# Bernat-C/MRI-Diffusion-SuperResolution

Hardware: AMD Instinct MI355X
Metric: MRI slices/sec (50-step DDIM, 256^2, bs=32) (higher is better)
Workload: dtype bf16; 1 GPU; configs[1]: 256x256 1-ch synthetic MRI slices -> 4x32x32 latents, SD-1.5-size UNet (859.5M params, random init) + rank-4 LoRA, 50-step DDIM, bs=32 per GPU; ddim_steps=50, parallelism=slice-sharded x1 (no collective), lora=explicit adapters, down-projection + rank-r update inside the projection GEMMs, tile_table=profiles/r03_tune_cache.tsv, hipgraph=True

## Files before the change

mri-diffusion-superresolution_amd/csrc/common.h:

```cpp
#pragma once
#include <hip/hip_runtime.h>
#include <stdint.h>
#include <string>

#include "lora_hr.h"

namespace mrisr {

typedef __bf16 bf16;
typedef __attribute__((ext_vector_type(8))) __bf16 bf16x8;
typedef __attribute__((ext_vector_type(4))) __bf16 bf16x4;
typedef __attribute__((ext_vector_type(4))) float f32x4;
typedef __attribute__((ext_vector_type(16))) float f32x16;

enum DType : int { DT_F32 = 0, DT_BF16 = 1, DT_F16 = 2, DT_I64 = 3 };

template <typename T> struct TypeTag;
template <> struct TypeTag<float> { static constexpr int id = DT_F32; };
template <> struct TypeTag<bf16> { static constexpr int id = DT_BF16; };

__device__ __forceinline__ float to_f32(float x) { return x; }
__device__ __forceinline__ float to_f32(bf16 x) { return (float)x; }
template <typename T> __device__ __forceinline__ T from_f32(float x);
template <> __device__ __forceinline__ float from_f32<float>(float x) { return x; }
// ... 97 lines not shown
    const float* lora_z = nullptr;
    const float* lora_b = nullptr;
    int lora_r = 0, lora_zld = 0, lora_secN = 1;
    const void* lora_a = nullptr;
    int lora_R = 0;
    float* lora_zout = nullptr;
    const float* ln_gamma = nullptr;
    const float* ln_beta = nullptr;
    float ln_eps = 1e-5f;
    const void* w8 = nullptr;
    const float* w_scale = nullptr;
    const void* lora_a8 = nullptr;
    const float* lora_a_scale = nullptr;
    int no_rp = 0;
    int group_m = 1;
    int dbg = 0;
    unsigned long long* stamps = nullptr;
};

template <typename T> int launch_gemm(const GemmArgs& g, hipStream_t st);
template <typename T> int launch_splitk_reduce(const GemmArgs& g, hipStream_t st);
const void* zero_page();
int init_zero_page();
int gemm_prepare();
struct MlpArgs {
    const void* x = nullptr; int ldx = 0, M = 0;
    const float* ln_gamma = nullptr; const float* ln_beta = nullptr; float ln_eps = 1e-5f;
    const void* w1 = nullptr; const float* b1 = nullptr;
    const void* w2p = nullptr; const float* b2 = nullptr;
    const void* resid = nullptr; int ldr = 0;
// ... 280 lines not shown
```

mri-diffusion-superresolution_amd/csrc/gemm.hip:

```cpp
#include "common.h"
#include "gemm_head.h"
#include "prof.h"

#include <cstdio>
#include <cstdlib>
#include <cstring>
#include <map>
#include <mutex>
#include <unordered_map>

namespace mrisr {

static void* g_zero_page = nullptr;
static constexpr size_t kZeroPageBytes = 128 * 1024;
const void* zero_page() { return g_zero_page; }
int init_zero_page() {
    if (g_zero_page) return 0;
    MRISR_CHECK_HIP(hipMalloc(&g_zero_page, kZeroPageBytes));
    MRISR_CHECK_HIP(hipMemset(g_zero_page, 0, kZeroPageBytes));
    return 0;
}

typedef const __attribute__((address_space(1))) void* gptr_t;
typedef __attribute__((address_space(3))) void* lptr_t;
// ... 172 lines not shown
template <int NFR>
__device__ __forceinline__ void preload_cols(const GemmArgs& g, int nbase, f32x4 (&pb)[NFR]) {
    const bool fold = g.rowvec && g.rowvec_div >= g.M;
#pragma unroll
    for (int i = 0; i < NFR; ++i) pb[i] = f32x4{0.f, 0.f, 0.f, 0.f};
    if (g.bias) {
#pragma unroll
        for (int i = 0; i < NFR; ++i) pb[i] = *reinterpret_cast<const f32x4*>(g.bias + min(nbase + i * 16, g.N - 4));
    }
    if (fold) {
#pragma unroll
        for (int i = 0; i < NFR; ++i) pb[i] += *reinterpret_cast<const f32x4*>(g.rowvec + min(nbase + i * 16, g.N - 4));
    }
}

template <typename T> struct Frag;
template <> struct Frag<bf16> { typedef bf16x8 type; };
template <> struct Frag<float> { typedef f32x4 type; };

__device__ __forceinline__ void mma(f32x4& acc, const bf16x8& w, const bf16x8& a) {
    acc = __builtin_amdgcn_mfma_f32_16x16x32_bf16(w, a, acc, 0, 0, 0);
}
__device__ __forceinline__ void mma(f32x4& acc, const f32x4& w, const f32x4& a) {
#pragma unroll
    for (int j = 0; j < 4; ++j) acc = __builtin_amdgcn_mfma_f32_16x16x4f32(w[j], a[j], acc, 0, 0, 0);
}

__device__ __forceinline__ void lds_poison(char* smem_base, int nthreads) {
    const unsigned bytes = ((const __attribute__((address_space(4))) unsigned*)__builtin_amdgcn_dispatch_ptr())[7];
    for (unsigned o = threadIdx.x * 16u; o + 16u <= bytes; o += (unsigned)nthreads * 16u)
        *reinterpret_cast<uint4*>(smem_base + o) = make_uint4(~0u, ~0u, ~0u, ~0u);
    __syncthreads();
}
static int gemm_flags_now();

static constexpr int kStampHdr = 8, kStampWgs = 1024, kStampSlotWords = kStampHdr + 8 * kStampWgs, kStampSlots = 256;
__device__ __forceinline__ unsigned long long* gemm_stamp_slot(const GemmArgs& g, bool header) {
    if (!g.stamps) return nullptr;
    const unsigned wg = blockIdx.x + gridDim.x * (blockIdx.y + gridDim.y * blockIdx.z);
    if (header && wg == 0 && threadIdx.x == 0) {
        g.stamps[0] = (unsigned long long)g.M; g.stamps[1] = (unsigned long long)g.N; g.stamps[2] = (unsigned long long)g.K;
        g.stamps[3] = (unsigned long long)gridDim.x * gridDim.y * gridDim.z;
        g.stamps[4] = (g.resid ? 1u : 0u) | (g.lora_a ? 2u : 0u) | (g.conv ? 4u : 0u) | (g.cs0 ? 8u : 0u);
        g.stamps[5] = (unsigned long long)g.splitk; g.stamps[6] = (unsigned long long)(unsigned)g.dbg; g.stamps[7] = 1ull;
    }
    return wg < (unsigned)kStampWgs ? g.stamps + kStampHdr + (size_t)wg * 8 : nullptr;
}
__device__ __forceinline__ unsigned long long* gemm_stamp_word(const GemmArgs& g, int k, bool header = false) {
    unsigned long long* const slot = gemm_stamp_slot(g, header);
    return slot ? slot + k : nullptr;
}
static_assert(kStampSlotWords == kStampHdr + 8 * kStampWgs, "a slot: the header, then 8 words for each of the first kStampWgs workgroups");

template <typename T, int BM, int BN, int WGM, int WGN>
__global__ __launch_bounds__(256) void gemm_kernel(const GemmArgs g, const char* __restrict__ zero) {
    constexpr int EB = sizeof(T);
    constexpr int CH = 16 / EB;
    constexpr int BK = 8 * CH;
// ... 205 lines not shown
#pragma unroll
    for (int i = 0; i < NF; ++i)
#pragma unroll
        for (int j = 0; j < MF; ++j) {
            const int m = m0 + wm0 + j * 16 + fr;
            const int n = n0 + wn0 + i * 16 + fg * 4;
            if (m < g.M && n < g.N) {
                float v[4] = {acc[i][j][0], acc[i][j][1], acc[i][j][2], acc[i][j][3]};
                epilogue4<T>(g, z, m, n, v, nullptr, nullptr, nullptr, false, true, nullptr, 0, 0, 0, pb[i]);
            }
        }
}

template <int BM, int BN, int NT = 256>
__device__ __forceinline__ void copy_out_tile(const GemmArgs& g, const bf16* otile, int pitch, int m0, int n0, int z, bool add_resid,
                                              unsigned long long* stamp_resid = nullptr) {
    __syncthreads();
    constexpr int CPR = BN / 8;
    bf16* out = reinterpret_cast<bf16*>(g.out) + (size_t)z * g.o_bs;
    const bf16* res = add_resid ? reinterpret_cast<const bf16*>(g.resid) + (size_t)z * g.o_bs : nullptr;
    constexpr int TOTAL = BM * CPR, IT = (TOTAL + NT - 1) / NT, BATCH = IT < 5 ? IT : 5;
    for (int it0 = 0; it0 < IT; it0 += BATCH) {
        bf16x8 rv[BATCH];
#pragma unroll
        for (int u = 0; u < BATCH; ++u) {
            const int idx = (int)threadIdx.x + (it0 + u) * NT;
            const int row = idx / CPR, ch = idx - row * CPR;
            const int m = m0 + row, n = n0 + ch * 8;
            if (res && idx < TOTAL && m < g.M && n + 8 <= g.N) rv[u] = *reinterpret_cast<const bf16x8*>(res + (size_t)m * g.ldr + n);
        }
        if (stamp_resid && it0 == 0 && threadIdx.x == 0) {
            if (res) asm volatile("s_waitcnt vmcnt(0)" ::: "memory");
            *stamp_resid = __builtin_readcyclecounter();
        }
#pragma unroll
        for (int u = 0; u < BATCH; ++u) {
            const int idx = (int)threadIdx.x + (it0 + u) * NT;
            const int row = idx / CPR, ch = idx - row * CPR;
            const int m = m0 + row, n = n0 + ch * 8;
            if (idx >= TOTAL || m >= g.M || n >= g.N) continue;
            const bf16* src = otile + row * pitch + ch * 8;
            bf16* dst = out + (size_t)m * g.ldo + n;
            if (n + 8 <= g.N) {
                bf16x8 v = *reinterpret_cast<const bf16x8*>(src);
                if (res) {
#pragma unroll
                    for (int e = 0; e < 8; ++e) v[e] = (bf16)((float)v[e] + (float)rv[u][e]);
// ... 38 lines not shown
            const int b = m / g.ntok, tok = m - b * g.ntok;
            *reinterpret_cast<bf16x8*>(base + (((size_t)b * g.nheads + h) * g.dpad + dd) * g.npad + tok) =
                *reinterpret_cast<const bf16x8*>(otile + col * P + tc * 8);
        }
    }
}

typedef __attribute__((address_space(3))) void* lds_ptr_t;
__device__ __forceinline__ __amdgpu_buffer_rsrc_t make_rsrc(const void* p, unsigned bytes) {
    return __builtin_amdgcn_make_buffer_rsrc(const_cast<void*>(p), 0, bytes, 0x00020000);
}
__device__ __forceinline__ void bl16(__amdgpu_buffer_rsrc_t r, char* lds_wave_base, unsigned voff, unsigned soff) {
    __builtin_amdgcn_raw_ptr_buffer_load_lds(r, (lds_ptr_t)lds_wave_base, 16, voff, soff, 0, 0);
}
#define BL_OOB 0x80000000u


__device__ __forceinline__ void pretouch_weights(const __amdgpu_buffer_rsrc_t& rw, long long w_bytes, char* scratch, int wave, int lane, int cap) {
    const int n_wg = (int)(gridDim.x * gridDim.y);
    const int wg = (int)(blockIdx.x + blockIdx.y * gridDim.x);
    const long long pieces = (w_bytes + 1023) >> 10;
    const int per_wg = (int)((pieces + n_wg - 1) / n_wg);
    const int per_wave = min((per_wg + 3) >> 2, cap);
    const long long first = (long long)wg * per_wg + (long long)wave * per_wave;
    for (int i = 0; i < per_wave; ++i) {
        const long long pc = first + i;
        const unsigned off = pc < pieces ? (unsigned)(pc << 10) + (unsigned)lane * 16u : BL_OOB;
        bl16(rw, scratch + ((wave * 2 + (i & 1)) << 10), off, 0u);
    }
}
// ... 218 lines not shown
                for (int it = 0; it < A_IT; ++it) bl16(rs, sb + (it * 256 + wave * 64) * 16, avo[it], chb);
            } else if (!second) {
#pragma unroll
                for (int it = 0; it < A_IT; ++it) bl16(ra0, sb + (it * 256 + wave * 64) * 16, avo[it], chb);
            } else {
#pragma unroll
                for (int it = 0; it < A_IT; ++it) bl16(ra1, sb + (it * 256 + wave * 64) * 16, avo[it], chb);
            }
            cc += BK;
            if (cc >= Ct && !tail) { cc = 0; ++tap; }
        }
    };
    auto stage = [&](int kt, int buf) { stage_w(kt, buf); stage_a(kt, buf); };
    (void)acb;
    if (kt_beg < kt_end) stage_a(kt_beg, 0);
    stamp(1);

    f32x4 acc[NF][MF];
#pragma unroll
    for (int i = 0; i < NF; ++i)
#pragma unroll
        for (int j = 0; j < MF; ++j) acc[i][j] = f32x4{0.f, 0.f, 0.f, 0.f};

    const int wm0 = (wave / WGN) * WTM, wn0 = (wave % WGN) * WTN;
    const int fr = lane & 15, fg = lane >> 4;
    const bool zwave = LORA && (wave % WGN) == 0;
    const bool lora_mma = LORA && g.lora_r == 4 && g.alpha == 1.0f && !(g.dbg & 8);
    bf16x8 lbf[NF];
    if (LORA) {
#pragma unroll
// ... 31 lines not shown
#pragma unroll
                for (int j = 0; j < MF; ++j) acc[i][j] = __builtin_amdgcn_mfma_f32_16x16x32_bf16(wf[i], af[j], acc[i][j], 0, 0, 0);
            if (LORA && zwave) {
                const bf16x8 lf = *reinterpret_cast<const bf16x8*>(sw + (BN + fr) * 128 + phys);
#pragma unroll
                for (int j = 0; j < MF; ++j) zacc[j] = __builtin_amdgcn_mfma_f32_16x16x32_bf16(lf, af[j], zacc[j], 0, 0, 0);
            }
        }
    };

    if constexpr (NSTAGE == 2) {
        if (kt_beg < kt_end) {
            asm volatile("s_waitcnt vmcnt(0)" ::: "memory");
            __syncthreads();
            stamp(2);
            int cur = 0;
            const bool halves = (g.dbg & 16384) != 0;
            for (int kt = kt_beg; kt < kt_end; ++kt) {
                const bool more = kt + 1 < kt_end;
                if (more) { if (halves) stage_w(kt + 1, cur ^ 1); else stage(kt + 1, cur ^ 1); }
                compute(cur, [&]() {
                    if (halves) {
                        __builtin_amdgcn_sched_barrier(0);
                        if (more) stage_a(kt + 1, cur ^ 1);
                        __builtin_amdgcn_sched_barrier(0);
                    }
                });
                asm volatile("s_waitcnt vmcnt(0)" ::: "memory");
                __syncthreads();
                cur ^= 1;
// ... 64 lines not shown
                    store4<float>(part + (size_t)m * g.N + n, v);
                }
            }
        if constexpr (NF * MF > 20) return;
        else {
            if (!g.sk_counters) return;
            if (!splitk_last_arriver<NF, MF>(g, acc, (unsigned)(z * gridDim.x + blockIdx.x), g.partial + (size_t)z * g.splitk * (size_t)g.M * g.N,
                                             m0 + wm0, n0 + wn0, fr, fg, smem))
                return;
        }
    }
    constexpr bool kRing = NSTAGE > 2;
    f32x4 pb[kRing ? 1 : NF];
    float pbr[kRing ? NF : 1][4];
    if constexpr (kRing) preload_cols<NF>(g, n0 + wn0 + fg * 4, pbr);
    else preload_cols<NF>(g, n0 + wn0 + fg * 4, pb);
    auto cols = [&](int i, float (&o)[4]) {
#pragma unroll
        for (int r = 0; r < 4; ++r) {
            if constexpr (kRing) o[r] = pbr[i][r];
            else o[r] = pb[i][r];
        }
    };
    stamp(4, true);
    if (g.act == ACT_GEGLU) {
        if constexpr (NF % 2 == 0) {
#pragma unroll
            for (int i = 0; i < NF; i += 2)
#pragma unroll
                for (int j = 0; j < MF; ++j) {
                    const int m = m0 + wm0 + j * 16 + fr;
// ... 49 lines not shown
#pragma unroll
            for (int j = 0; j < MF; ++j) {
                const int m = m0 + wm0 + j * 16 + fr;
                const int n = n0 + wn0 + i * 16 + fg * 4;
                if (m < g.M && n < g.N) {
                    float v[4] = {acc[i][j][0], acc[i][j][1], acc[i][j][2], acc[i][j][3]};
                    float pbi[4];
                    cols(i, pbi);
                    epilogue4<T>(g, z, m, n, v, nullptr, LORA && !lora_mma ? zlds + (m - m0) * 16 : nullptr,
                                 staged || (hstaged && !htr) ? otile + (m - m0) * OPITCH + (n - n0) : nullptr, resid_later, true,
                                 hstaged && htr ? otile : nullptr, m - m0, n - n0, BM + 8, pbi);
                }
            }
    }
    stamp(5);
    if (staged) copy_out_tile<BM, BN>(g, otile, OPITCH, m0, n0, z, resid_later, NSTAGE == 2 ? gemm_stamp_word(g, 6) : nullptr);
    else if (hstaged) copy_out_heads<BM, BN>(g, otile, m0, n0, htr);
    stamp(7);
}

template <int BM, int BN, int WGM, int WGN>
__global__ __launch_bounds__(256, 2) void gemm_halo_kernel(const GemmHead hd, const GemmArgs g) {
    typedef bf16 T;
    constexpr int BK = 64;
    constexpr int W_IT = BN / 32;
    constexpr int WTM = BM / WGM, WTN = BN / WGN;
    constexpr int MF = WTM / 16, NF = WTN / 16;
    constexpr int WSTAGE = BN * 128;
    constexpr int PIT_MAX = (BM >= 256 ? 13 : (BM >= 128 ? 9 : 6));
    static_assert(WGM * WGN == 4, "4 waves");
    extern __shared__ __attribute__((aligned(16))) char smem[];
// ... 93 lines not shown
    }

    auto stage_patch = [&](int ch) {
        const int cc = ch * BK;
        const bool second = cc >= (int)h.c0;
        const unsigned chb = (unsigned)(second ? cc - (int)h.c0 : cc) * 2;
#pragma unroll
        for (int it = 0; it < PIT_MAX; ++it) {
            if (it < pit) {
                if (!second) bl16(ra0, patch + (it * 256 + wave * 64) * 16, pvo0[it], chb);
                else bl16(ra1, patch + (it * 256 + wave * 64) * 16, pvo1[it], chb);
            }
        }
    };
    if (ch_beg < ch_end) stage_patch(ch_beg);
    stamp(1);

    const bool has_tail = (h.flags & GH_TAIL) != 0;
    const long long a_rows = has_tail ? (long long)g.B * Hd * Wd : 0ll;
    const void* const s0p = has_tail ? g.s0 : nullptr;
    const void* const s1p = has_tail ? g.s1 : nullptr;
    const __amdgpu_buffer_rsrc_t rs0 = make_rsrc(s0p ? s0p : (const void*)a0p, s0p ? (unsigned)min(a_rows * g.lds0 * 2, 0x7FFFFFFFll) : 0u);
    const __amdgpu_buffer_rsrc_t rs1 = make_rsrc(s1p ? s1p : (const void*)a0p, s1p ? (unsigned)min(a_rows * g.lds1 * 2, 0x7FFFFFFFll) : 0u);
    unsigned spix[PIT_MAX];
    auto sc_setup = [&]() {
#pragma unroll
        for (int it = 0; it < PIT_MAX; ++it) {
            int t = it * 256 + tid;
            asm volatile("" : "+v"(t));
            const int pp = t >> 3;
// ... 68 lines not shown
                for (int t = tid; t < npix * 8; t += 256) {
                    bf16x8 v = *reinterpret_cast<bf16x8*>(patch + t * 16);
#pragma unroll
                    for (int e = 0; e < 8; ++e) {
                        const float f = (float)v[e] * 1.0009765625f + 0.03125f;
                        v[e] = (bf16)(f / (1.0f + __expf(-f)));
                    }
                    *reinterpret_cast<bf16x8*>(patch + t * 16) = v;
                }
                __syncthreads();
            }
            for (int tap = 0; tap < 9; ++tap) {
                if (tap + 1 < 9) stage_w(ch, tap + 1, cur ^ 1);
                else if (ch + 1 < ch_end) stage_w(ch + 1, 0, cur ^ 1);
                else if (sc_beg < sc_end) stage_w_sc(sc_beg, cur ^ 1);
                compute(cur, tap);
                asm volatile("s_waitcnt vmcnt(0)" ::: "memory");
                __syncthreads();
                cur ^= 1;
            }
        }
        if (sc_beg < sc_end) sc_setup();
        for (int sc = sc_beg; sc < sc_end; ++sc) {
            stage_patch_sc(sc);
            asm volatile("s_waitcnt vmcnt(0)" ::: "memory");
            __syncthreads();
            if (sc + 1 < sc_end) stage_w_sc(sc + 1, cur ^ 1);
            compute(cur, 4);
            asm volatile("s_waitcnt vmcnt(0)" ::: "memory");
            __syncthreads();
// ... 14 lines not shown
                    float v[4] = {acc[i][j][0], acc[i][j][1], acc[i][j][2], acc[i][j][3]};
                    store4<float>(part + (size_t)m * g.N + n, v);
                }
            }
        if constexpr (NF * MF > 20) return;
        else {
            if (!g.sk_counters) return;
            if (!splitk_last_arriver<NF, MF>(g, acc, blockIdx.x, g.partial, m0 + wm0, n0 + wn0, fr, fg, smem)) return;
        }
    }
    constexpr int OPITCH = BN + 8;
    T* otile = reinterpret_cast<T*>(smem);
    const bool staged = g.out_mode == OUT_ROWS && (g.ldo & 7) == 0 && (size_t)BM * OPITCH * 2 <= (size_t)pit * 4096 + 2 * WSTAGE && g.stage_out > 1;
    const bool resid_later = staged && g.resid != nullptr && (g.ldr & 7) == 0 && g.stage_out < 3;
    f32x4 pb[NF];
    preload_cols<NF>(g, n0 + wn0 + fg * 4, pb);
    stamp(4, true);
    const bool plain_epi = !(g.dbg & 64) && staged && g.act == ACT_NONE && !g.lora_z && (!g.resid || resid_later);
    if (plain_epi) {
        const float alpha = g.alpha;
        const bool rows_rv = g.rowvec && g.rowvec_div < g.M;
#pragma unroll
        for (int i = 0; i < NF; ++i)
#pragma unroll
            for (int j = 0; j < MF; ++j) {
                const int ml = wm0 + j * 16 + fr, nl = wn0 + i * 16 + fg * 4;
                if (m0 + ml < g.M && n0 + nl < g.N) {
                    f32x4 a = acc[i][j];
#pragma unroll
                    for (int r = 0; r < 4; ++r) a[r] = a[r] * alpha + pb[i][r];
                    if (rows_rv) a += *reinterpret_cast<const f32x4*>(g.rowvec + (size_t)((m0 + ml) / g.rowvec_div) * g.rowvec_ld + n0 + nl);
// ... 5 lines not shown
#pragma unroll
        for (int i = 0; i < NF; ++i)
#pragma unroll
            for (int j = 0; j < MF; ++j) {
                const int m = m0 + wm0 + j * 16 + fr;
                const int n = n0 + wn0 + i * 16 + fg * 4;
                if (m < g.M && n < g.N) {
                    float v[4] = {acc[i][j][0], acc[i][j][1], acc[i][j][2], acc[i][j][3]};
                    const float pbi[4] = {pb[i][0], pb[i][1], pb[i][2], pb[i][3]};
                    epilogue4<T>(g, 0, m, n, v, nullptr, nullptr, staged ? otile + (m - m0) * OPITCH + (n - n0) : nullptr, resid_later, true, nullptr,
                                 0, 0, 0, pbi);
                }
            }
    }
    stamp(5);
    if (staged) copy_out_tile<BM, BN>(g, otile, OPITCH, m0, n0, 0, resid_later, gemm_stamp_word(g, 6));
    stamp(7);
}

template <int BN, int NSTAGE>
__global__ __launch_bounds__(512, 2) void gemm_halo8_kernel(const GemmArgs g) {
    typedef bf16 T;
    constexpr int BM = 256, NT = 512, BK = 64, WGN = 2;
    constexpr int WTM = 64, WTN = BN / WGN;
    constexpr int MF = WTM / 16, NF = WTN / 16;
    constexpr int W_IT = (BN * 8 + NT - 1) / NT;
    constexpr int WSTAGE = W_IT * NT * 16;
    constexpr int PIT_MAX = 7;
    constexpr int D = NSTAGE - 1;
    static_assert(NSTAGE >= 2 && NSTAGE <= 4, "2..4 weight stages");
    extern __shared__ __attribute__((aligned(16))) char smem[];
// ... 1422 lines not shown
    ProfScope ps = gemm_scope(g, base, nullptr, g.conv ? conv_a_elements(g, false) : (double)g.M * g.K, sizeof(T), sizeof(T), st);
    hipLaunchKernelGGL(kern, grid, dim3(256), smem, st, g, (const char*)zero_page());
    MRISR_CHECK_HIP(hipGetLastError());
    return 0;
}

static GemmHead gemm_head_for(const GemmArgs& g, int BM, int BN, bool halo) {
    GemmHeadIn in;
    in.w = g.w; in.a0 = g.a0; in.a1 = g.a1;
    in.M = g.M; in.N = g.N; in.K = g.K; in.c0 = g.c0; in.c1 = g.c1; in.lda0 = g.lda0; in.lda1 = g.lda1;
    in.conv = g.conv; in.B = g.B; in.Hin = g.Hin; in.Win = g.Win; in.Hout = g.Hout; in.Wout = g.Wout;
    in.ups = g.ups; in.zstuff = g.zstuff; in.subpix = g.subpix;
    in.cs0 = g.cs0; in.cs1 = g.cs1; in.splitk = g.splitk; in.batch = g.batch; in.group_m = g.group_m;
    in.pretouch = g.pretouch; in.dbg = g.dbg; in.stamped = g.stamps != nullptr;
    in.BM = BM; in.BN = BN; in.halo = halo;
    return make_gemm_head(in);
}

static int g_force_tile = 0;
extern "C" void mrisr_debug_force_tile(int t) { g_force_tile = t; }

template <int BM, int BN, int WGM, int WGN, int NSTAGE>
static int prepare_bl() {
    constexpr int smem = NSTAGE * (BM + BN) * 128;
    constexpr int smem_l = NSTAGE * ((BM + BN) * 128 + 16 * 128);
    static bool done = false;
    if (!done) {
        MRISR_CHECK_HIP(hipFuncSetAttribute((const void*)gemm_bl_kernel<BM, BN, WGM, WGN, NSTAGE, false>, hipFuncAttributeMaxDynamicSharedMemorySize, smem));
        MRISR_CHECK_HIP(hipFuncSetAttribute((const void*)gemm_bl_kernel<BM, BN, WGM, WGN, NSTAGE, true>, hipFuncAttributeMaxDynamicSharedMemorySize, smem_l));
        done = true;
    }
    return 0;
}
template <int BM, int BN, int WGM, int WGN, int NSTAGE>
static int launch_bl(GemmArgs& g, hipStream_t st) {
    constexpr int smem = NSTAGE * (BM + BN) * 128;
    constexpr int smem_l = NSTAGE * ((BM + BN) * 128 + 16 * 128);
    if (prepare_bl<BM, BN, WGM, WGN, NSTAGE>()) return 1;
    const dim3 grid = tile_grid(g, BM, BN);
    static const std::string base = std::string("gemm_bf16_bl") + std::to_string(BM) + "x" + std::to_string(BN) + (NSTAGE > 2 ? "d" + std::to_string(NSTAGE) : std::string());
    ProfScope ps = gemm_scope(g, base, g.conv ? (g.cs0 ? "convsc" : (g.ups ? "convup" : (g.stride == 2 ? "convs2" : "conv"))) : "lin",
                              g.conv ? conv_a_elements(g, true) : (double)g.M * g.K, 2, 2, st);
    const GemmHead hd = gemm_head_for(g, BM, BN, false);
    if (g.lora_a) hipLaunchKernelGGL((gemm_bl_kernel<BM, BN, WGM, WGN, NSTAGE, true>), grid, dim3(256), smem_l, st, hd, g);
    else hipLaunchKernelGGL((gemm_bl_kernel<BM, BN, WGM, WGN, NSTAGE, false>), grid, dim3(256), smem, st, hd, g);
    MRISR_CHECK_HIP(hipGetLastError());
    return 0;
}

static size_t halo_smem(const GemmArgs& g, int BM, int BN) {
    const int TH = BM / g.Win;
    const size_t npix = (size_t)(TH + 2) * (g.Win + 2);
    const size_t patch = (npix * 8 + 255) / 256 * 4096;
    return patch + 2 * (size_t)BN * 128;
}
template <int BM, int BN, int WGM, int WGN>
static int launch_halo(GemmArgs& g, hipStream_t st) {
    const size_t smem = halo_smem(g, BM, BN);
    MRISR_REQUIRE(smem <= 160 * 1024, "halo conv kernel: LDS");
    static size_t attr = 0;
    if (smem > attr) {
        MRISR_CHECK_HIP(hipFuncSetAttribute((const void*)gemm_halo_kernel<BM, BN, WGM, WGN>, hipFuncAttributeMaxDynamicSharedMemorySize, (int)(96 * 1024)));
        attr = 96 * 1024;
    }
    const dim3 grid = tile_grid(g, BM, BN);
    static const std::string base = std::string("gemm_bf16_halo") + std::to_string(BM) + "x" + std::to_string(BN);
    ProfScope ps = gemm_scope(g, base, g.cs0 ? "convsc" : "conv", conv_a_elements(g, true), 2, 2, st);
    hipLaunchKernelGGL((gemm_halo_kernel<BM, BN, WGM, WGN>), grid, dim3(256), smem, st, gemm_head_for(g, BM, BN, true), g);
    MRISR_CHECK_HIP(hipGetLastError());
    return 0;
}
template <int BN, int NSTAGE>
static int launch_halo8(GemmArgs& g, hipStream_t st) {
    const int npix = (256 / g.Win + 2) * (g.Win + 2);
    const size_t smem = (size_t)((npix * 8 + 511) / 512) * 8192 + (size_t)NSTAGE * ((BN * 8 + 511) / 512) * 8192;
    MRISR_REQUIRE(smem <= 160 * 1024, "256-row halo conv kernel: LDS");
    static bool attr = false;
    if (!attr) {
// ... 517 lines not shown
```

mri-diffusion-superresolution_amd/csrc/gemm_head.h:

```cpp
#pragma once
#include <cstdint>

#if defined(__HIPCC__) || defined(__CUDACC__)
#define MRISR_GH_HD __host__ __device__ __forceinline__
#else
#define MRISR_GH_HD inline
#endif

namespace mrisr {

struct MagicDiv {
    uint32_t mul;
    uint32_t l;
};
inline MagicDiv magic_for(uint32_t d) {
    MagicDiv m{0x80000000u, 0u};
    if (d <= 1) return m;
    uint32_t l = 0;
    while ((1ull << l) < d) ++l;
    m.l = l;
    m.mul = (uint32_t)(((1ull << (31 + l)) + d - 1) / d);
    return m;
}
MRISR_GH_HD uint32_t magic_div(uint32_t x, uint32_t mul, uint32_t l) { return (uint32_t)(((uint64_t)x * mul) >> (31u + l)); }

enum : uint32_t {
    GH_DBG_MASK = 0xFFFFu,
    GH_CONV = 1u << 16,
    GH_SUBPIX = 1u << 17,
    GH_ZSTUFF = 1u << 18,
    GH_UPS = 1u << 19,
    GH_A1 = 1u << 20,
    GH_TAIL = 1u << 21,
    GH_STAMPED = 1u << 22,
    GH_BATCHED = 1u << 23,
};
enum { GH_SH_PG = 0, GH_SH_GM = 5, GH_SH_LAST = 10, GH_SH_HW = 15, GH_SH_WD = 20, GH_SH_PW = 25 };

struct GemmHead {
    const void* w;
    const void* a0;
    const void* a1;
    uint32_t ext_w, ext_a0, ext_a1;
    uint32_t flags;
    uint32_t rows;
    uint32_t N;
    uint32_t wpitch;
    uint32_t lda0, lda1;
    uint32_t c0;
    uint32_t ntn, ntm;
// ... 5 lines not shown
    uint32_t pt_per_wg, pt_per_wave;
    uint32_t mul_hw, mul_wd, mul_pw;
    uint32_t geom;
    uint32_t per_sc;
};
static_assert(sizeof(GemmHead) == 128, "the head is two 64-byte lines");

MRISR_GH_HD uint32_t gh_shift(const GemmHead& h, int field) { return (h.shifts >> field) & 31u; }

struct GemmHeadIn {
    const void *w = nullptr, *a0 = nullptr, *a1 = nullptr;
    int M = 0, N = 0, K = 0, c0 = 0, c1 = 0, lda0 = 0, lda1 = 0;
    int conv = 0, B = 0, Hin = 0, Win = 0, Hout = 0, Wout = 0, ups = 0, zstuff = 0, subpix = 0;
    int cs0 = 0, cs1 = 0, splitk = 1, batch = 1, group_m = 1, pretouch = 0, dbg = 0, stamped = 0;
    int BM = 64, BN = 64, halo = 0;
};

static inline uint32_t gh_clamp_extent(long long bytes) { return (uint32_t)(bytes < 0x7FFFFFFFll ? bytes : 0x7FFFFFFFll); }

inline GemmHead make_gemm_head(const GemmHeadIn& in) {
    GemmHead h{};
    h.w = in.w; h.a0 = in.a0; h.a1 = in.a1;
    const long long a_rows = in.conv ? (long long)in.B * in.Hin * in.Win : (long long)in.M;
    h.ext_w = gh_clamp_extent((long long)in.N * in.K * 2);
    h.ext_a0 = gh_clamp_extent(a_rows * in.lda0 * 2);
    h.ext_a1 = in.a1 ? gh_clamp_extent(a_rows * in.lda1 * 2) : 0u;
    h.flags = ((uint32_t)in.dbg & GH_DBG_MASK) | (in.conv ? GH_CONV : 0u) | (in.subpix ? GH_SUBPIX : 0u) | (in.zstuff ? GH_ZSTUFF : 0u) |
              (in.ups ? GH_UPS : 0u) | (in.a1 ? GH_A1 : 0u) | (in.cs0 ? GH_TAIL : 0u) | (in.stamped ? GH_STAMPED : 0u) |
              (in.batch > 1 ? GH_BATCHED : 0u);
    h.rows = (uint32_t)(in.halo ? in.Hin : in.M);
    h.N = (uint32_t)in.N;
    h.wpitch = (uint32_t)in.K * 2u;
    h.lda0 = (uint32_t)in.lda0; h.lda1 = (uint32_t)in.lda1; h.c0 = (uint32_t)in.c0;
    h.ntn = (uint32_t)((in.N + in.BN - 1) / in.BN);
    h.ntm = (uint32_t)(in.halo ? in.M / in.BM : (in.M + in.BM - 1) / in.BM);
    const uint32_t GM = (uint32_t)(in.group_m > 1 ? in.group_m : 1);
    h.group_m = GM;
    const uint32_t last = h.ntm % GM ? h.ntm % GM : GM;
    const MagicDiv pg = magic_for(GM * h.ntn), gm = magic_for(GM), ls = magic_for(last);
    h.mul_pg = pg.mul; h.mul_gm = gm.mul; h.mul_last = ls.mul;
    const int Ct = in.c0 + in.c1;
    h.Ct = (uint32_t)Ct;
    const int units = in.halo ? Ct / 64 : in.K / 64;
    h.per = (uint32_t)((units + in.splitk - 1) / in.splitk);
// ... 7 lines not shown
        h.pt_per_wave = (uint32_t)(per_wave < in.pretouch ? per_wave : in.pretouch);
    }
    MagicDiv hw = magic_for(1), wd = magic_for(1), pw = magic_for(1);
    if (in.halo) {
        const int TH = in.BM / in.Win, PW = in.Win + 2, npix = (TH + 2) * PW, pit = (npix * 8 + 255) / 256;
        hw = magic_for((uint32_t)(in.Hin * in.Win)); wd = magic_for((uint32_t)in.Win); pw = magic_for((uint32_t)PW);
        h.geom = (uint32_t)in.Win | (uint32_t)TH << 8 | (uint32_t)PW << 16 | (uint32_t)pit << 24;
    } else if (in.conv) {
        hw = magic_for((uint32_t)(in.Hout * in.Wout)); wd = magic_for((uint32_t)in.Wout);
    }
    h.mul_hw = hw.mul; h.mul_wd = wd.mul; h.mul_pw = pw.mul;
    h.shifts = pg.l << GH_SH_PG | gm.l << GH_SH_GM | ls.l << GH_SH_LAST | hw.l << GH_SH_HW | wd.l << GH_SH_WD | pw.l << GH_SH_PW;
    return h;
}

MRISR_GH_HD void gh_tile_coords(const GemmHead& h, uint32_t bid, uint32_t& tm, uint32_t& tn) {
    const uint32_t nblk = h.ntn * h.ntm;
    const uint32_t xcd = bid & 7u, q = nblk >> 3, r = nblk & 7u;
    const uint32_t logical = (xcd < r ? xcd * (q + 1u) : r * (q + 1u) + (xcd - r) * q) + (bid >> 3);
    const uint32_t per_group = h.group_m * h.ntn;
    const uint32_t grp = magic_div(logical, h.mul_pg, gh_shift(h, GH_SH_PG));
    const uint32_t first_m = grp * h.group_m;
    const uint32_t left = h.ntm - first_m;
    const bool full = h.group_m <= left;
    const uint32_t gsz = full ? h.group_m : left;
    const uint32_t within = logical - grp * per_group;
    tn = magic_div(within, full ? h.mul_gm : h.mul_last, gh_shift(h, full ? GH_SH_GM : GH_SH_LAST));
    tm = first_m + (within - tn * gsz);
}
MRISR_GH_HD void gh_split_range(uint32_t per, uint32_t total, uint32_t split, int& beg, int& end) {
// ... 15 lines not shown
```

Measured before the change: 72.60 slices/s.

## Prefetch bias/rowvec and residual tiles into LDS during GEMM mainloop

Adds optional LDS regions past the staging buffers. Bias and rowvec columns, and the residual tile, are loaded asynchronously with buffer-to-LDS loads early in the bl and halo GEMM kernels. The epilogue then reads them from LDS instead of issuing global loads after the K loop, hiding that epilogue memory latency behind compute. A host-side planner enables each region only when the extra LDS keeps the same workgroups per CU, the kernel finishes the tile (no unreduced split-K), and shape and alignment constraints hold. Dynamic LDS sizing changes, and residual loads compete with mainloop traffic.

```diff
diff --git a/mri-diffusion-superresolution_amd/csrc/common.h b/mri-diffusion-superresolution_amd/csrc/common.h
--- a/mri-diffusion-superresolution_amd/csrc/common.h
+++ b/mri-diffusion-superresolution_amd/csrc/common.h
@@ -135,6 +135,7 @@
     const float* lora_a_scale = nullptr;
     int no_rp = 0;
     int group_m = 1;
+    int epi_lds = 0;
     int dbg = 0;
     unsigned long long* stamps = nullptr;
 };
diff --git a/mri-diffusion-superresolution_amd/csrc/gemm.hip b/mri-diffusion-superresolution_amd/csrc/gemm.hip
--- a/mri-diffusion-superresolution_amd/csrc/gemm.hip
+++ b/mri-diffusion-superresolution_amd/csrc/gemm.hip
@@ -210,6 +210,23 @@
     }
 }
 
+template <int NFR>
+__device__ __forceinline__ void preload_cols(const GemmArgs& g, const char* cols, int nl, int nbase, f32x4 (&pb)[NFR]) {
+    const bool fold = g.rowvec && g.rowvec_div >= g.M;
+#pragma unroll
+    for (int i = 0; i < NFR; ++i) pb[i] = f32x4{0.f, 0.f, 0.f, 0.f};
+    if (g.bias) {
+#pragma unroll
+        for (int i = 0; i < NFR; ++i)
+            pb[i] = *(cols ? reinterpret_cast<const f32x4*>(cols + (nl + i * 16) * 4) : reinterpret_cast<const f32x4*>(g.bias + min(nbase + i * 16, g.N - 4)));
+    }
+    if (fold) {
+#pragma unroll
+        for (int i = 0; i < NFR; ++i)
+            pb[i] += *(cols ? reinterpret_cast<const f32x4*>(cols + 1024 + (nl + i * 16) * 4) : reinterpret_cast<const f32x4*>(g.rowvec + min(nbase + i * 16, g.N - 4)));
+    }
+}
+
 template <typename T> struct Frag;
 template <> struct Frag<bf16> { typedef bf16x8 type; };
 template <> struct Frag<float> { typedef f32x4 type; };
@@ -237,7 +254,7 @@
     if (header && wg == 0 && threadIdx.x == 0) {
         g.stamps[0] = (unsigned long long)g.M; g.stamps[1] = (unsigned long long)g.N; g.stamps[2] = (unsigned long long)g.K;
         g.stamps[3] = (unsigned long long)gridDim.x * gridDim.y * gridDim.z;
-        g.stamps[4] = (g.resid ? 1u : 0u) | (g.lora_a ? 2u : 0u) | (g.conv ? 4u : 0u) | (g.cs0 ? 8u : 0u);
+        g.stamps[4] = (g.resid ? 1u : 0u) | (g.lora_a ? 2u : 0u) | (g.conv ? 4u : 0u) | (g.cs0 ? 8u : 0u) | ((unsigned)(g.epi_lds & 3) << 4);
         g.stamps[5] = (unsigned long long)g.splitk; g.stamps[6] = (unsigned long long)(unsigned)g.dbg; g.stamps[7] = 1ull;
     }
     return wg < (unsigned)kStampWgs ? g.stamps + kStampHdr + (size_t)wg * 8 : nullptr;
@@ -473,7 +490,7 @@
 
 template <int BM, int BN, int NT = 256>
 __device__ __forceinline__ void copy_out_tile(const GemmArgs& g, const bf16* otile, int pitch, int m0, int n0, int z, bool add_resid,
-                                              unsigned long long* stamp_resid = nullptr) {
+                                              unsigned long long* stamp_resid = nullptr, const char* res_lds = nullptr) {
     __syncthreads();
     constexpr int CPR = BN / 8;
     bf16* out = reinterpret_cast<bf16*>(g.out) + (size_t)z * g.o_bs;
@@ -486,10 +503,11 @@
             const int idx = (int)threadIdx.x + (it0 + u) * NT;
             const int row = idx / CPR, ch = idx - row * CPR;
             const int m = m0 + row, n = n0 + ch * 8;
-            if (res && idx < TOTAL && m < g.M && n + 8 <= g.N) rv[u] = *reinterpret_cast<const bf16x8*>(res + (size_t)m * g.ldr + n);
+            if (res && idx < TOTAL && m < g.M && n + 8 <= g.N)
+                rv[u] = *(res_lds ? reinterpret_cast<const bf16x8*>(res_lds + idx * 16) : reinterpret_cast<const bf16x8*>(res + (size_t)m * g.ldr + n));
         }
         if (stamp_resid && it0 == 0 && threadIdx.x == 0) {
-            if (res) asm volatile("s_waitcnt vmcnt(0)" ::: "memory");
+            if (res) asm volatile("s_waitcnt vmcnt(0) lgkmcnt(0)" ::: "memory");
             *stamp_resid = __builtin_readcyclecounter();
         }
 #pragma unroll
@@ -558,6 +576,31 @@
     __builtin_amdgcn_raw_ptr_buffer_load_lds(r, (lds_ptr_t)lds_wave_base, 16, voff, soff, 0, 0);
 }
 #define BL_OOB 0x80000000u
+
+__device__ __forceinline__ void cols_to_lds(const GemmArgs& g, char* cols, int n0, unsigned N, int wave, int lane) {
+    const unsigned voff = (unsigned)(n0 + 4 * lane) * 4u;
+    if (wave == 0) {
+        const float* const b = g.bias;
+        if (b) bl16(make_rsrc(b, N * 4u), cols, voff, 0u);
+    } else if (wave == 1) {
+        const float* const t = g.rowvec;
+        if (t && g.rowvec_div >= g.M) bl16(make_rsrc(t, N * 4u), cols + 1024, voff, 0u);
+    }
+}
+template <int BM, int BN>
+__device__ __forceinline__ void resid_to_lds(const GemmArgs& g, char* region, int m0, int n0, int tid, int wave, int it_lo, int it_hi) {
+    constexpr int CPR = BN / 8, TOTAL = BM * CPR;
+    const unsigned M = (unsigned)g.M, N = (unsigned)g.N, ldr2 = (unsigned)g.ldr * 2u;
+    const __amdgpu_buffer_rsrc_t rr = make_rsrc(g.resid, M * ldr2);
+    for (int it = it_lo; it < it_hi; ++it) {
+        int idx = tid + it * 256;
+        asm volatile("" : "+v"(idx));
+        const int row = idx / CPR, ch = idx - row * CPR;
+        const unsigned m = (unsigned)(m0 + row), n = (unsigned)(n0 + ch * 8);
+        const bool ok = idx < TOTAL && m < M && n + 8u <= N;
+        bl16(rr, region + (it * 256 + wave * 64) * 16, ok ? m * ldr2 + n * 2u : BL_OOB, 0u);
+    }
+}
 
 
 __device__ __forceinline__ void pretouch_weights(const __amdgpu_buffer_rsrc_t& rw, long long w_bytes, char* scratch, int wave, int lane, int cap) {
@@ -806,6 +849,16 @@
     auto stage = [&](int kt, int buf) { stage_w(kt, buf); stage_a(kt, buf); };
     (void)acb;
     if (kt_beg < kt_end) stage_a(kt_beg, 0);
+    constexpr int COLS_OFF = epi_bl_stage_bytes(BM, BN, NSTAGE, LORA), RES_OFF = COLS_OFF + kEpiColsBytes;
+    constexpr bool kResFits = epi_bl_resid_may_fit(BM, BN, NSTAGE, LORA);
+    constexpr int RES_IT = epi_resid_rounds(BM, BN);
+    static_assert(BN <= 256 && epi_out_tile_bytes(BM, BN, LORA) <= COLS_OFF, "a column piece covers the tile; z rows and output tile stay inside the stages");
+    if constexpr (NSTAGE == 2) {
+        if (h.flags & GH_COLS_LDS) cols_to_lds(g, smem + COLS_OFF, n0, h.N, wave, lane);
+        if constexpr (kResFits) {
+            if ((h.flags & GH_RESID_LDS) && kt_beg + 1 >= kt_end) resid_to_lds<BM, BN>(g, smem + RES_OFF, m0, n0, tid, wave, 0, RES_IT);
+        }
+    }
     stamp(1);
 
     f32x4 acc[NF][MF];
@@ -867,6 +920,9 @@
             asm volatile("s_waitcnt vmcnt(0)" ::: "memory");
             __syncthreads();
             stamp(2);
+            if constexpr (kResFits) {
+                if (kt_beg + 1 < kt_end && (h.flags & GH_RESID_LDS)) resid_to_lds<BM, BN>(g, smem + RES_OFF, m0, n0, tid, wave, 0, RES_IT);
+            }
             int cur = 0;
             const bool halves = (g.dbg & 16384) != 0;
             for (int kt = kt_beg; kt < kt_end; ++kt) {
@@ -961,7 +1017,7 @@
     f32x4 pb[kRing ? 1 : NF];
     float pbr[kRing ? NF : 1][4];
     if constexpr (kRing) preload_cols<NF>(g, n0 + wn0 + fg * 4, pbr);
-    else preload_cols<NF>(g, n0 + wn0 + fg * 4, pb);
+    else preload_cols<NF>(g, (g.epi_lds & 1) ? smem + COLS_OFF : nullptr, wn0 + fg * 4, n0 + wn0 + fg * 4, pb);
     auto cols = [&](int i, float (&o)[4]) {
 #pragma unroll
         for (int r = 0; r < 4; ++r) {
@@ -1041,7 +1097,8 @@
             }
     }
     stamp(5);
-    if (staged) copy_out_tile<BM, BN>(g, otile, OPITCH, m0, n0, z, resid_later, NSTAGE == 2 ? gemm_stamp_word(g, 6) : nullptr);
+    if (staged) copy_out_tile<BM, BN>(g, otile, OPITCH, m0, n0, z, resid_later, NSTAGE == 2 ? gemm_stamp_word(g, 6) : nullptr,
+                                      kResFits && (g.epi_lds & 2) ? smem + RES_OFF : nullptr);
     else if (hstaged) copy_out_heads<BM, BN>(g, otile, m0, n0, htr);
     stamp(7);
 }
@@ -1165,6 +1222,11 @@
         }
     };
     if (ch_beg < ch_end) stage_patch(ch_beg);
+    constexpr bool kResFits = epi_halo_resid_may_fit(BM, BN);
+    constexpr int RES_IT = epi_resid_rounds(BM, BN);
+    static_assert(BN <= 256, "a column piece covers the tile");
+    char* const cols_lds = wbase + 2 * WSTAGE;
+    if (h.flags & GH_COLS_LDS) cols_to_lds(g, cols_lds, n0, h.N, wave, lane);
     stamp(1);
 
     const bool has_tail = (h.flags & GH_TAIL) != 0;
@@ -1263,6 +1325,9 @@
                 if (tap + 1 < 9) stage_w(ch, tap + 1, cur ^ 1);
                 else if (ch + 1 < ch_end) stage_w(ch + 1, 0, cur ^ 1);
                 else if (sc_beg < sc_end) stage_w_sc(sc_beg, cur ^ 1);
+                if constexpr (kResFits) {
+                    if (tap == 0 && ch == ch_beg && (h.flags & GH_RESID_LDS)) resid_to_lds<BM, BN>(g, wbase + 2 * WSTAGE + kEpiColsBytes, m0, n0, tid, wave, 0, RES_IT);
+                }
                 compute(cur, tap);
                 asm volatile("s_waitcnt vmcnt(0)" ::: "memory");
                 __syncthreads();
@@ -1307,7 +1372,7 @@
     const bool staged = g.out_mode == OUT_ROWS && (g.ldo & 7) == 0 && (size_t)BM * OPITCH * 2 <= (size_t)pit * 4096 + 2 * WSTAGE && g.stage_out > 1;
     const bool resid_later = staged && g.resid != nullptr && (g.ldr & 7) == 0 && g.stage_out < 3;
     f32x4 pb[NF];
-    preload_cols<NF>(g, n0 + wn0 + fg * 4, pb);
+    preload_cols<NF>(g, (g.epi_lds & 1) ? wbase + 2 * WSTAGE : nullptr, wn0 + fg * 4, n0 + wn0 + fg * 4, pb);
     stamp(4, true);
     const bool plain_epi = !(g.dbg & 64) && staged && g.act == ACT_NONE && !g.lora_z && (!g.resid || resid_later);
     if (plain_epi) {
@@ -1343,7 +1408,8 @@
             }
     }
     stamp(5);
-    if (staged) copy_out_tile<BM, BN>(g, otile, OPITCH, m0, n0, 0, resid_later, gemm_stamp_word(g, 6));
+    if (staged) copy_out_tile<BM, BN>(g, otile, OPITCH, m0, n0, 0, resid_later, gemm_stamp_word(g, 6),
+                                      kResFits && (g.epi_lds & 2) ? wbase + 2 * WSTAGE + kEpiColsBytes : nullptr);
     stamp(7);
 }
 
@@ -2796,7 +2862,23 @@
     in.cs0 = g.cs0; in.cs1 = g.cs1; in.splitk = g.splitk; in.batch = g.batch; in.group_m = g.group_m;
     in.pretouch = g.pretouch; in.dbg = g.dbg; in.stamped = g.stamps != nullptr;
     in.BM = BM; in.BN = BN; in.halo = halo;
+    in.cols_lds = g.epi_lds & 1; in.resid_lds = g.epi_lds & 2;
     return make_gemm_head(in);
+}
+static EpiLds epi_lds_for(GemmArgs& g, int BM, int BN, int nstage, bool halo, bool in_kernel_reduce, bool staged_rows) {
+    EpiLdsIn in;
+    in.BM = BM; in.BN = BN; in.nstage = nstage; in.lora = g.lora_a != nullptr; in.halo = halo; in.Win = g.Win;
+    in.M = g.M; in.N = g.N; in.ldr = g.ldr; in.batch = g.batch;
+    in.finishes = g.splitk == 1 || (g.sk_counters != nullptr && in_kernel_reduce);
+    in.k_units = halo ? (g.c0 + g.c1) / 64 : g.K / 64;
+    in.splitk = g.splitk;
+    in.has_cols = g.bias != nullptr || (g.rowvec != nullptr && g.rowvec_div >= g.M);
+    in.geglu = g.act == ACT_GEGLU;
+    in.resid_later = staged_rows && g.resid != nullptr && (g.ldr & 7) == 0 && g.stage_out < 3;
+    in.dbg = g.dbg;
+    const EpiLds e = epi_lds_plan(in);
+    g.epi_lds = (e.cols ? 1 : 0) | (e.resid ? 2 : 0);
+    return e;
 }
 
 static int g_force_tile = 0;
@@ -2804,8 +2886,8 @@
 
 template <int BM, int BN, int WGM, int WGN, int NSTAGE>
 static int prepare_bl() {
-    constexpr int smem = NSTAGE * (BM + BN) * 128;
-    constexpr int smem_l = NSTAGE * ((BM + BN) * 128 + 16 * 128);
+    constexpr int smem = epi_bl_max_bytes(BM, BN, NSTAGE, false);
+    constexpr int smem_l = epi_bl_max_bytes(BM, BN, NSTAGE, true);
     static bool done = false;
     if (!done) {
         MRISR_CHECK_HIP(hipFuncSetAttribute((const void*)gemm_bl_kernel<BM, BN, WGM, WGN, NSTAGE, false>, hipFuncAttributeMaxDynamicSharedMemorySize, smem));
@@ -2816,10 +2898,11 @@
 }
 template <int BM, int BN, int WGM, int WGN, int NSTAGE>
 static int launch_bl(GemmArgs& g, hipStream_t st) {
-    constexpr int smem = NSTAGE * (BM + BN) * 128;
-    constexpr int smem_l = NSTAGE * ((BM + BN) * 128 + 16 * 128);
     if (prepare_bl<BM, BN, WGM, WGN, NSTAGE>()) return 1;
     const dim3 grid = tile_grid(g, BM, BN);
+    constexpr bool reduces = (BM / WGM / 16) * (BN / WGN / 16) <= 20;
+    const bool staged = g.out_mode == OUT_ROWS && (g.ldo & 7) == 0 && g.heads == 1 && g.stage_out;
+    const size_t smem = (size_t)epi_lds_for(g, BM, BN, NSTAGE, false, reduces, staged).total, smem_l = smem;
     static const std::string base = std::string("gemm_bf16_bl") + std::to_string(BM) + "x" + std::to_string(BN) + (NSTAGE > 2 ? "d" + std::to_string(NSTAGE) : std::string());
     ProfScope ps = gemm_scope(g, base, g.conv ? (g.cs0 ? "convsc" : (g.ups ? "convup" : (g.stride == 2 ? "convs2" : "conv"))) : "lin",
                               g.conv ? conv_a_elements(g, true) : (double)g.M * g.K, 2, 2, st);
@@ -2838,12 +2921,19 @@
 }
 template <int BM, int BN, int WGM, int WGN>
 static int launch_halo(GemmArgs& g, hipStream_t st) {
-    const size_t smem = halo_smem(g, BM, BN);
-    MRISR_REQUIRE(smem <= 160 * 1024, "halo conv kernel: LDS");
+    const size_t stages = halo_smem(g, BM, BN);
+    MRISR_REQUIRE(stages <= 160 * 1024, "halo conv kernel: LDS");
+    constexpr int OPITCH = BN + 8;
+    constexpr bool reduces = (BM / WGM / 16) * (BN / WGN / 16) <= 20;
+    const bool staged = g.out_mode == OUT_ROWS && (g.ldo & 7) == 0 && (size_t)BM * OPITCH * 2 <= stages && g.stage_out > 1;
+    const EpiLds el = epi_lds_for(g, BM, BN, 2, true, reduces, staged);
+    MRISR_REQUIRE((size_t)el.stage_bytes == stages, "halo conv kernel: LDS layout");
+    const size_t smem = (size_t)el.total;
     static size_t attr = 0;
     if (smem > attr) {
-        MRISR_CHECK_HIP(hipFuncSetAttribute((const void*)gemm_halo_kernel<BM, BN, WGM, WGN>, hipFuncAttributeMaxDynamicSharedMemorySize, (int)(96 * 1024)));
-        attr = 96 * 1024;
+        const size_t want = std::max(smem, (size_t)96 * 1024);
+        MRISR_CHECK_HIP(hipFuncSetAttribute((const void*)gemm_halo_kernel<BM, BN, WGM, WGN>, hipFuncAttributeMaxDynamicSharedMemorySize, (int)want));
+        attr = want;
     }
     const dim3 grid = tile_grid(g, BM, BN);
     static const std::string base = std::string("gemm_bf16_halo") + std::to_string(BM) + "x" + std::to_string(BN);
diff --git a/mri-diffusion-superresolution_amd/csrc/gemm_head.h b/mri-diffusion-superresolution_amd/csrc/gemm_head.h
--- a/mri-diffusion-superresolution_amd/csrc/gemm_head.h
+++ b/mri-diffusion-superresolution_amd/csrc/gemm_head.h
@@ -34,6 +34,8 @@
     GH_TAIL = 1u << 21,
     GH_STAMPED = 1u << 22,
     GH_BATCHED = 1u << 23,
+    GH_COLS_LDS = 1u << 24,
+    GH_RESID_LDS = 1u << 25,
 };
 enum { GH_SH_PG = 0, GH_SH_GM = 5, GH_SH_LAST = 10, GH_SH_HW = 15, GH_SH_WD = 20, GH_SH_PW = 25 };
 
@@ -69,6 +71,7 @@
     int conv = 0, B = 0, Hin = 0, Win = 0, Hout = 0, Wout = 0, ups = 0, zstuff = 0, subpix = 0;
     int cs0 = 0, cs1 = 0, splitk = 1, batch = 1, group_m = 1, pretouch = 0, dbg = 0, stamped = 0;
     int BM = 64, BN = 64, halo = 0;
+    int cols_lds = 0, resid_lds = 0;
 };
 
 static inline uint32_t gh_clamp_extent(long long bytes) { return (uint32_t)(bytes < 0x7FFFFFFFll ? bytes : 0x7FFFFFFFll); }
@@ -82,7 +85,7 @@
     h.ext_a1 = in.a1 ? gh_clamp_extent(a_rows * in.lda1 * 2) : 0u;
     h.flags = ((uint32_t)in.dbg & GH_DBG_MASK) | (in.conv ? GH_CONV : 0u) | (in.subpix ? GH_SUBPIX : 0u) | (in.zstuff ? GH_ZSTUFF : 0u) |
               (in.ups ? GH_UPS : 0u) | (in.a1 ? GH_A1 : 0u) | (in.cs0 ? GH_TAIL : 0u) | (in.stamped ? GH_STAMPED : 0u) |
-              (in.batch > 1 ? GH_BATCHED : 0u);
+              (in.batch > 1 ? GH_BATCHED : 0u) | (in.cols_lds ? GH_COLS_LDS : 0u) | (in.resid_lds ? GH_RESID_LDS : 0u);
     h.rows = (uint32_t)(in.halo ? in.Hin : in.M);
     h.N = (uint32_t)in.N;
     h.wpitch = (uint32_t)in.K * 2u;
@@ -120,6 +123,66 @@
     return h;
 }
 
+constexpr int kLdsPerCU = 160 * 1024, kEpiColsBytes = 2048;
+enum { EPI_COLS_OFF = 32, EPI_RESID_OFF = 256 };
+constexpr int epi_bl_stage_bytes(int BM, int BN, int nstage, bool lora) { return nstage * ((BM + BN) * 128 + (lora ? 16 * 128 : 0)); }
+constexpr int epi_halo_patch_bytes(int BM, int Win) { return (((BM / Win + 2) * (Win + 2) * 8 + 255) / 256) * 4096; }
+constexpr int epi_halo_stage_bytes(int BM, int BN, int Win) { return epi_halo_patch_bytes(BM, Win) + 2 * BN * 128; }
+constexpr int epi_resid_rounds(int BM, int BN) { return (BM * (BN / 8) + 255) / 256; }
+constexpr int epi_resid_bytes(int BM, int BN) { return epi_resid_rounds(BM, BN) * 4096; }
+constexpr int epi_out_tile_bytes(int BM, int BN, bool lora) { return BM * (BN + 8) * 2 + (lora ? BM * 64 : 0); }
+constexpr int epi_wg_per_cu(int lds_bytes) { return lds_bytes <= 0 ? 0 : kLdsPerCU / lds_bytes; }
+constexpr bool epi_keeps_wgs(int base, int with_regions) { return epi_wg_per_cu(base) >= 2 && epi_wg_per_cu(with_regions) == epi_wg_per_cu(base); }
+
+struct EpiLdsIn {
+    int BM = 64, BN = 64, nstage = 2, lora = 0, halo = 0, Win = 0;
+    long long M = 0;
+    int N = 0, ldr = 0, batch = 1;
+    int finishes = 1;
+    int k_units = 1, splitk = 1;
+    int has_cols = 0;
+    int geglu = 0;
+    int resid_later = 0;
+    int dbg = 0;
+};
+struct EpiLds {
+    int stage_bytes = 0;
+    int cols_off = 0, resid_off = 0;
+    int resid_bytes = 0;
+    int total = 0;
+    bool cols = false, resid = false;
+};
+inline EpiLds epi_lds_plan(const EpiLdsIn& in) {
+    EpiLds e;
+    e.stage_bytes = in.halo ? epi_halo_stage_bytes(in.BM, in.BN, in.Win) : epi_bl_stage_bytes(in.BM, in.BN, in.nstage, in.lora != 0);
+    e.cols_off = e.stage_bytes;
+    e.resid_off = e.cols_off + kEpiColsBytes;
+    e.resid_bytes = epi_resid_bytes(in.BM, in.BN);
+    e.total = e.stage_bytes;
+    if (in.nstage != 2 || !in.finishes || in.BN > 256) return e;
+    const int per = (in.k_units + in.splitk - 1) / (in.splitk > 0 ? in.splitk : 1);
+    if (in.k_units < 1 || in.splitk < 1 || (long long)(in.splitk - 1) * per >= in.k_units) return e;
+    const bool fits_cols = epi_keeps_wgs(e.stage_bytes, e.resid_off);
+    const bool fits_resid = epi_keeps_wgs(e.stage_bytes, e.resid_off + e.resid_bytes);
+    e.cols = fits_cols && in.has_cols && !in.geglu && !(in.dbg & EPI_COLS_OFF) && (in.N & 3) == 0 && in.N < (1 << 29);
+    e.resid = fits_resid && in.resid_later && in.batch == 1 && (in.N & 7) == 0 && (in.ldr & 7) == 0 && in.ldr >= in.N &&
+              in.M * (long long)in.ldr * 2 < 0x7FFFFFFFll && !(in.dbg & EPI_RESID_OFF);
+    if (e.cols || e.resid) e.total = e.resid_off + (e.resid ? e.resid_bytes : 0);
+    return e;
+}
+constexpr int epi_bl_max_bytes(int BM, int BN, int nstage, bool lora) {
+    const int base = epi_bl_stage_bytes(BM, BN, nstage, lora);
+    if (nstage != 2 || !epi_keeps_wgs(base, base + kEpiColsBytes)) return base;
+    const int all = base + kEpiColsBytes + epi_resid_bytes(BM, BN);
+    return epi_keeps_wgs(base, all) ? all : base + kEpiColsBytes;
+}
+constexpr bool epi_bl_resid_may_fit(int BM, int BN, int nstage, bool lora) {
+    return nstage == 2 && epi_bl_max_bytes(BM, BN, nstage, lora) > epi_bl_stage_bytes(BM, BN, nstage, lora) + kEpiColsBytes;
+}
+constexpr bool epi_halo_resid_may_fit(int BM, int BN) {
+    return 2 * (4096 + 2 * BN * 128 + kEpiColsBytes + epi_resid_bytes(BM, BN)) <= kLdsPerCU;
+}
+
 MRISR_GH_HD void gh_tile_coords(const GemmHead& h, uint32_t bid, uint32_t& tm, uint32_t& tn) {
     const uint32_t nblk = h.ntn * h.ntm;
     const uint32_t xcd = bid & 7u, q = nblk >> 3, r = nblk & 7u;
```

New measurement: 72.35 slices/s. Within noise of the previous version (-0.3%).
